# Mariachiar/Spatiotemporal-Deepfake-Detection-for-Live-Video-Calls

Measured on AMD Instinct MI355X. Metric: clips/sec (32x3x224x224), higher is better.
Workload: dtype bf16

## Files before the change

### spatiotemporal-deepfake-detection-for-live-video-calls_amd/csrc/af_conv.hip

```cpp
#include "af_common.h"
#include <stdlib.h>

namespace af {

#ifdef AF_STAMPS
#define AF_STAMP_DECL unsigned long long stamp_v[8] = {0, 0, 0, 0, 0, 0, 0, 0}
#define AF_DBG(bit) (a.dbg & (bit))
#define AF_STAMP(slot) stamp_v[slot] = (slot) >= 6 ? __builtin_amdgcn_s_memrealtime() : __builtin_amdgcn_s_memtime()
#define AF_STAMP_FLUSH do { if (a.stamps && lane < 8) a.stamps[((long long)bid * 8 + wave) * 8 + lane] = \
    lane == 0 ? stamp_v[0] : lane == 1 ? stamp_v[1] : lane == 2 ? stamp_v[2] : lane == 3 ? stamp_v[3] : lane == 4 ? stamp_v[4] : lane == 5 ? stamp_v[5] : lane == 6 ? stamp_v[6] : stamp_v[7]; } while (0)
#else
#define AF_STAMP_DECL do {} while (0)
#define AF_DBG(bit) false
#define AF_STAMP(slot) do {} while (0)
#define AF_STAMP_FLUSH do {} while (0)
#endif

struct ConvArgs {
    const char* in;
    const char* w;
    const float* scale;
    const float* shift;
    const char* res;
    char* out;
// ... 569 lines not shown
    conv_igemm_tile<DT, BN, BM, WN, WM, KS, NSTAGE, MINW, DUAL, SPLITK, BMR>(a, blockIdx.x, gridDim.x);
}

template <int DT, int BN, int BM, int WN, int WM, int KS, int MINW, bool DUAL, int NSTAGE = 3, bool SPLITK = false, int BMR = BM>
static int launch(const ConvArgs& a, hipStream_t stream) {
    const long long tiles_m = (a.M + BMR - 1) / BMR;
    const long long blocks = tiles_m * a.tiles_n;
    if (blocks <= 0 || blocks > 0x7fffffffLL) return set_error(AF_ERR_ARG, "conv: grid of %lld workgroups", blocks);
    constexpr int TMv = BMR / WM / 16;
    constexpr int red_bytes = KS == 2 ? WN * WM * (BN / WN / 16) * TMv * 64 * 16 : 0;
    constexpr int patch_bytes = red_bytes + WN * WM * ((TMv % 4 == 0 && TMv >= 8 ? TMv / 4 : TMv % 2 == 0 ? TMv / 2 : 1) * 16) * (BN / WN + 4) * 4;
    const int S = a.kt * a.kh * a.kw * a.kpt + a.kpt2;
    const int slots = (MINW >= 4 && a.ring == 2) ? 2 : NSTAGE;
    const int ring_bytes = (S < slots ? S : slots) * (BN + BM) * 128;
    const int lds = ring_bytes > patch_bytes ? ring_bytes : patch_bytes;
    AF_SET_MAX_LDS((&conv_igemm_kernel<DT, BN, BM, WN, WM, KS, NSTAGE, MINW, DUAL, SPLITK, BMR>),
                   NSTAGE * (BN + BM) * 128 > patch_bytes ? NSTAGE * (BN + BM) * 128 : patch_bytes, "conv");
    hipLaunchKernelGGL((conv_igemm_kernel<DT, BN, BM, WN, WM, KS, NSTAGE, MINW, DUAL, SPLITK, BMR>), dim3((unsigned)blocks, SPLITK ? a.ksplit : 1), dim3(WN * WM * KS * 64), lds, stream, a);
    AF_CHECK_LAUNCH("conv_igemm_kernel");
    return AF_OK;
}

enum { VAR_128x256 = 0, VAR_64x256 = 1, VAR_128x128 = 2, VAR_64x128 = 3, VAR_C133 = 4, VAR_128x128_R2 = 5, VAR_256x256 = 6,
       VAR_128x512 = 7, VAR_C311 = 8, VAR_SMALL = 9, VAR_C111 = 10, VAR_C133G = 11, VAR_256x224 = 12, VAR_C311G = 13, VAR_COUNT = 14 };
static const char* const kVariantNames[] = {"conv_igemm<BN=128,BM=256>", "conv_igemm<BN=64,BM=256>",
                                            "conv_igemm<BN=128,BM=128>", "conv_igemm<BN=64,BM=128>",
                                            "conv133_c64<weights in registers>", "conv_igemm<BN=128,BM=128>",
                                            "conv_igemm<BN=256,BM=256>", "conv_igemm<BN=128,BM=512>",
                                            "conv311_c64<time-tiled, taps share one LDS image>",
                                            "conv_small<direct-gather MFMA, narrow layers>",
                                            "conv111<persistent stream, weights in registers>",
                                            "conv133g<frame-resident halo patch, 9 taps share it>",
                                            "conv_igemm<BN=256,BM=224>",
                                            "conv311g<clip-resident (T + 2) x P patch, 3 taps share it>"};

static int pick_variant(int cout, int cin, int taps, int dtype, long long M, int cin2 = 0, int pooled = 0) {
    if (const char* fv = getenv("AF_FORCE_VAR")) {
        const int v = atoi(fv);
        const int bn = (v == VAR_256x256 || v == VAR_256x224) ? 256 : (v == VAR_128x256 || v == VAR_128x512 || v == VAR_128x128 || v == VAR_128x128_R2) ? 128 : 64;
        const bool generic = v == VAR_128x256 || v == VAR_64x256 || v == VAR_128x128 || v == VAR_64x128 || v == VAR_128x128_R2 ||
                             v == VAR_256x256 || v == VAR_128x512 || v == VAR_256x224;
        if (generic && cout % bn == 0 && !(pooled && v == VAR_256x224)) return v;
    }
    const int ksteps = (taps * cin + cin2) / (dtype == AF_F32 ? 32 : 64);
    const bool wide = cout % 128 == 0, short_k = ksteps <= 3;
    if (cout % 256 == 0 && ksteps >= (pooled == 2 ? 4 : cin2 ? 6 : 9)) {
        const char* e224 = getenv("AF_IGEMM_224");
        const int mode224 = e224 ? atoi(e224) : 1;
        const long long tm = (M + 255) / 256, big = tm * (cout / 256), v0 = tm * (cout / 128);
        const long long b224 = (M + 223) / 224 * (cout / 256);
        const double c256 = (double)((big + 255) / 256), c224 = 0.89 * (double)((b224 + 255) / 256);
        const bool take224 = pooled == 0 && mode224 != 0 && (mode224 == 2 || (M % 49 == 0 && c224 < c256 - 0.02));
        if (big >= 128 && (take224 ? c224 : c256) < 0.615 * (double)((v0 + 255) / 256) + 0.05) return take224 ? VAR_256x224 : VAR_256x256;
    }
    if (cout == 128 && !cin2 && taps >= 9) {
        const long long big = (M + 511) / 512, v0 = (M + 255) / 256;
        if (big >= 128 && (double)((big + 255) / 256) < 0.615 * (double)((v0 + 255) / 256) + 0.05) return VAR_128x512;
// ... 73 lines not shown
            case VAR_256x224: rc = launch<DT, 256, 256, 4, 2, 1, 2, false, 2, false, 224>(a, stream); break;
            case VAR_128x512: rc = launch<DT, 128, 512, 2, 4, 1, 2, false, 2>(a, stream); break;
            case VAR_128x256: rc = launch<DT, 128, 256, 2, 4, 1, 2, false>(a, stream); break;
            case VAR_64x256: rc = launch<DT, 64, 256, 1, 8, 1, 2, false>(a, stream); break;
            case VAR_128x128:
            case VAR_128x128_R2: rc = launch<DT, 128, 128, 2, 4, 1, 6, false>(a, stream); break;
            default: rc = launch<DT, 64, 128, 1, 8, 1, 4, false>(a, stream); break;
        }
    }
    if (rc != AF_OK || a.ksplit == 1) return rc;
    const long long quads = a.M * (a.Cout / 4);
    hipLaunchKernelGGL((splitk_finish_kernel<DT>), dim3((unsigned)((quads + 255) / 256)), dim3(256), 0, stream, a.ws, a.ksplit, a.M, a.Cout,
                       a.scale, a.shift, a.res, a.relu, a.out, a.out_ld);
    AF_CHECK_LAUNCH("splitk_finish_kernel");
    return AF_OK;
}

}

extern "C" int af_conv_variant(const af_conv_desc* d, const af_conv_desc* d2) {
    AF_REQUIRE(d && d->cout > 0 && d->cin > 0 && af::dtype_ok(d->dtype), "conv_variant: bad descriptor");
    if (af::conv_small_applies(d, d2, nullptr, 0)) return af::VAR_SMALL;
    if (!d2 && af::conv133_applies(d, nullptr, 0)) return af::VAR_C133;
    if (!d2 && af::conv133g_applies(d, nullptr, 0)) return af::VAR_C133G;
    if (!d2 && af::conv311g_applies(d, nullptr, 0)) return af::VAR_C311G;
    if (!d2 && af::conv311_applies(d, nullptr, 0)) return af::VAR_C311;
    if (af::conv111_applies(d, d2, nullptr, 0)) return af::VAR_C111;
    const int bk = d->dtype == AF_F32 ? 32 : 64;
    return af::pick_variant((d->cout + 63) / 64 * 64, (d->cin + bk - 1) / bk * bk, d->kt * d->kh * d->kw, d->dtype,
                            (long long)d->n * d->to * d->ho * d->wo, d2 ? (d2->cin + bk - 1) / bk * bk : 0, d->tpool);
}

extern "C" const char* af_conv_variant_name(int variant) {
    return (variant >= 0 && variant < af::VAR_COUNT) ? af::kVariantNames[variant] : "?";
}

extern "C" int64_t af_conv_workspace_bytes(const af_conv_desc* d) {
    using namespace af;
    if (!d || d->cout <= 0 || d->cin <= 0 || !dtype_ok(d->dtype) || d->n <= 0 || d->to <= 0 || d->ho <= 0 || d->wo <= 0) return 0;
    const int bk = d->dtype == AF_F32 ? 32 : 64;
    const int coutp = (d->cout + 63) / 64 * 64, cinp = (d->cin + bk - 1) / bk * bk, taps = d->kt * d->kh * d->kw;
    const long long M = (long long)d->n * d->to * d->ho * d->wo;
    const int v = pick_variant(coutp, cinp, taps, d->dtype, M, 0, d->tpool);
    const int ks = plan_ksplit(v, M, coutp, d->cout, taps * (cinp / bk), d->tpool, false);
    return ks > 1 ? (int64_t)ks * M * d->cout * (int64_t)sizeof(float) : 0;
}

// ... 146 lines not shown
```

### spatiotemporal-deepfake-detection-for-live-video-calls_amd/csrc/af_conv133g.hip

```cpp
#include "af_common.h"
#include <stdlib.h>

namespace af {

#ifdef AF_STAMPS
#define AF_STAMP_DECL unsigned long long stamp_v[8] = {0, 0, 0, 0, 0, 0, 0, 0}
#define AF_DBG(bit) (a.dbg & (bit))
#define AF_STAMP(slot) stamp_v[slot] = (slot) >= 6 ? __builtin_amdgcn_s_memrealtime() : __builtin_amdgcn_s_memtime()
#define AF_STAMP_FLUSH do { if (a.stamps && lane < 8) a.stamps[((long long)blockIdx.x * 8 + wave) * 8 + lane] = \
    lane == 0 ? stamp_v[0] : lane == 1 ? stamp_v[1] : lane == 2 ? stamp_v[2] : lane == 3 ? stamp_v[3] : lane == 4 ? stamp_v[4] : lane == 5 ? stamp_v[5] : lane == 6 ? stamp_v[6] : stamp_v[7]; } while (0)
#else
#define AF_STAMP_DECL do {} while (0)
#define AF_DBG(bit) false
#define AF_STAMP(slot) do {} while (0)
#define AF_STAMP_FLUSH do {} while (0)
#endif

struct C133GArgs {
    const char* in;
    const char* w;
    const float* scale;
    const float* shift;
    char* out;
    int H, W, Cin, Cout, frames;
    int T, kt;
    int R, upf;
    int WP;
    int prows;
    int kslabs;
    int relu, out_ld;
    float inv_wp;
    const char* w2;
    const float* scale2;
    const float* shift2;
    const char* res;
    int Cout2, relu2;
    int stagger;
#ifdef AF_STAMPS
    unsigned long long* stamps;
    int dbg;
#endif
};

template <int DT, int WN, int WM, int MT, bool FUSEC, int MAXP, int NSLOT, bool TEMPORAL>
__global__ __launch_bounds__(512, 2) void conv133g_kernel(const C133GArgs a) {
    typedef Elem<DT> E;
    typedef typename E::type OT;
    static_assert(E::EPC == 8 && WN * WM == 8, "16-bit operands, 8 waves");
    constexpr int NT = 4;
    constexpr int BN = WN * 64;
    constexpr int RW = BN / 64;
    constexpr int WSTAGE = BN * 128;
    constexpr int PROW = 64 + 8;
    constexpr int NTAPS = TEMPORAL ? 3 : 9;
    constexpr int PSTEPS = TEMPORAL ? NTAPS - 1 : NTAPS;
    constexpr int PPS = (MAXP + PSTEPS - 1) / PSTEPS;
    static_assert(!(TEMPORAL && FUSEC) && NSLOT <= NTAPS, "temporal mode: no fused c conv; the prologue's stages are taps of slab 0");

    extern __shared__ uint4 smem[];
    const unsigned lds0 = (unsigned)(uintptr_t)(__attribute__((address_space(3))) char*)smem;
    const int tid = threadIdx.x, lane = tid & 63;
    const int wave = __builtin_amdgcn_readfirstlane(tid >> 6);
    const int wn = wave % WN, wm = wave / WN;
    const int frow = lane & 15, fg = lane >> 4;
    const int WP = a.WP;
    const int pbytes = a.prows * 128;
    const unsigned ring0 = lds0 + 2 * pbytes;

    const int units = a.frames * a.upf;
    int unit = blockIdx.x;
    int frame = unit / a.upf, h0 = (unit - frame * a.upf) * a.R;
    const int HW = a.H * a.W;
    const int lrow = tid >> 3, wchunk = (tid & 7) ^ (lrow & 7);
    const long long Kw = (long long)NTAPS * a.kt * a.Cin;
    const i32x4 wdesc = make_desc(a.w);
    const unsigned woff = (unsigned)((lrow * Kw + wchunk * 8) * 2);
    const int wpiece_bytes = (int)(64 * Kw * 2);
    const int NP = a.prows >> 3;
    const int pt = a.kt >> 1;
    int tclip = frame % a.T;
    const int frame_bytes = a.H * a.W * a.Cin * 2;
    auto unit_desc = [&]() {
        return make_desc(TEMPORAL ? a.in + ((((long long)frame * a.T - 1) * HW + h0) * a.Cin) * 2
                                  : a.in + ((((long long)frame - pt) * a.H + h0 - 1) * a.W) * a.Cin * 2);
    };
    i32x4 xdesc = unit_desc();
    constexpr bool POFF_LDS = WN == 2;
    unsigned poff[POFF_LDS ? 1 : MAXP];
    const unsigned tab0 = ring0 + NSLOT * WSTAGE;
    const unsigned tabl = tab0 + (unsigned)((wave * 8 + (lane >> 3)) * 4);
    const unsigned pchunk16 = (unsigned)(((lane & 7) ^ (lane >> 3)) * 16);
    auto patch_slab_offset = [&](int ks, bool& inclip) {
        const int dt = (ks >= a.kslabs) + (ks >= 2 * a.kslabs), cs = ks - dt * a.kslabs;
        inclip = (unsigned)(tclip + dt - pt) < (unsigned)a.T;
        return __builtin_amdgcn_readfirstlane(dt * frame_bytes + cs * 128);
    };
    auto issue_patch_piece = [&](int bufoff, int soff, bool inclip, int i, unsigned voff) {
        if (wave + 8 * i < NP)
            blds16_m0(inclip ? voff : kOutOfRange, xdesc, soff, __builtin_amdgcn_readfirstlane(lds0 + bufoff + (wave + 8 * i) * 1024));
    };
    auto table_offset = [&](unsigned word) { return word == kOutOfRange ? kOutOfRange : word + pchunk16; };
    auto w_slab_offset = [&](int ks) {
        const int dt = (ks >= a.kslabs) + (ks >= 2 * a.kslabs), cs = ks - dt * a.kslabs;
        return __builtin_amdgcn_readfirstlane((dt * NTAPS * a.Cin + cs * 64) * 2);
    };
    const int tap_bytes = a.Cin * 2;
    auto issue_w_piece = [&](int stoff, int soff, int i) {
        blds16_m0(woff, wdesc, soff + i * wpiece_bytes, __builtin_amdgcn_readfirstlane(ring0 + stoff + (64 * i + 8 * wave) * 128));
    };

    f32x4 acc[NT][MT];

    const int nslabs = a.kt * a.kslabs;
    AF_STAMP_DECL;
    AF_STAMP(0); AF_STAMP(6);
    auto row_offset = [&](int j) -> unsigned {
        if (TEMPORAL) {
            const int tf = (int)(((float)j + 0.5f) * a.inv_wp), q = j - tf * a.R;
            const bool ok = tf >= 1 && tf <= a.T && h0 + q < HW;
            return ok ? (unsigned)((((long long)tf * HW + q) * a.Cin) * 2) : kOutOfRange;
        }
        const int q = j - 1;
        const int r = (int)(((float)q + 0.5f) * a.inv_wp), c = q - r * WP;
        const bool ok = q >= 0 && r < a.R + 2 && c >= 1 && c <= a.W && (unsigned)(h0 - 1 + r) < (unsigned)a.H;
        return ok ? (unsigned)(((r * a.W + (c - 1)) * a.Cin) * 2) : kOutOfRange;
    };
    auto compute_poff = [&]() {
        if constexpr (POFF_LDS) {
            int t = tid;
            asm volatile("" : "+v"(t));
            unsigned* tab = reinterpret_cast<unsigned*>(reinterpret_cast<char*>(smem) + (tab0 - lds0));
            for (int j = t; j < a.prows; j += 512) tab[j] = row_offset(j);
            asm volatile("s_waitcnt lgkmcnt(0)" ::: "memory");
            __builtin_amdgcn_s_barrier();
        } else {
            int drow = lane >> 3;
            asm volatile("" : "+v"(drow));
#pragma unroll
            for (int i = 0; i < MAXP; ++i) poff[i] = table_offset(row_offset((wave + 8 * i) * 8 + drow));
        }
    };
    auto issue_unit_head = [&](int bufoff) {
#pragma unroll
        for (int k = 0; k < NSLOT; ++k)
#pragma unroll
            for (int i = 0; i < RW; ++i) issue_w_piece(k * WSTAGE, w_slab_offset(0) + k * tap_bytes, i);
        compute_poff();
        bool in0;
        const int ps0 = patch_slab_offset(0, in0);
        if constexpr (POFF_LDS) {
            unsigned w[MAXP];
            static_for<MAXP>([&](auto i) { w[i] = lds_read4_uncounted<i * 256>(tabl); });
            wait_lgkmcnt<0>();
#pragma unroll
            for (int i = 0; i < MAXP; ++i) { asm volatile("" : "+v"(w[i])); issue_patch_piece(bufoff, ps0, in0, i, table_offset(w[i])); }
        } else {
#pragma unroll
            for (int i = 0; i < MAXP; ++i) issue_patch_piece(bufoff, ps0, in0, i, poff[i]);
        }
    };
    issue_unit_head(0);
    int bstart = 0;
    const unsigned arow = ring0 + (wn * 64 + frow) * 128, brow = lds0 + (wm * MT * 16 + frow) * 128;
    u32x4 a0[NT], b0[MT], a1[NT], b1[MT];
    auto frag_read = [&](u32x4 (&af)[NT], u32x4 (&bf)[MT], unsigned wsb, unsigned xsb, auto idx) {
        constexpr int r = decltype(idx)::value;
        if constexpr (r < NT) af[r] = lds_read16_uncounted<r * (16 * 128)>(wsb);
        else if constexpr (r < NT + MT) bf[r - NT] = lds_read16_uncounted<(r - NT) * (16 * 128)>(xsb);
    };
    auto w_addr = [&](int stoff, int kk) { return arow + stoff + ((((kk << 2) + fg) ^ (frow & 7)) << 4); };
    auto x_addr = [&](int bufoff, int sh, int kk) { return brow + bufoff + sh * 128 + ((((kk << 2) + fg) ^ ((frow + sh) & 7)) << 4); };
    auto pin_half = [&](u32x4 (&af)[NT], u32x4 (&bf)[MT]) {
#pragma unroll
        for (int i = 0; i < NT; ++i) pin_frag(af[i]);
#pragma unroll
        for (int j = 0; j < MT; ++j) pin_frag(bf[j]);
    };
    constexpr int NTH = NT * MT, NR = NT + MT;
    auto mma_group = [&](auto t0c, auto t1c, auto rlimc, const u32x4 (&af)[NT], const u32x4 (&bf)[MT], u32x4 (&naf)[NT], u32x4 (&nbf)[MT],
                         unsigned wsb, unsigned xsb) {
        constexpr int T0 = decltype(t0c)::value, T1 = decltype(t1c)::value, RLIM = decltype(rlimc)::value;
// ... 18 lines not shown
    for (;;) {
    wait_vmcnt<0>();
    __builtin_amdgcn_s_barrier();
#pragma unroll
    for (int i = 0; i < NT; ++i)
#pragma unroll
        for (int j = 0; j < MT; ++j) { acc[i][j] = f32x4{0.f, 0.f, 0.f, 0.f}; acc_live(acc[i][j]); }
    mfma_operands_settled();
    {
        constexpr int H1 = 3 * NTH / 4;
        static_assert(NR + RW + PPS <= NTH, "a DMA piece or a read per MFMA of the second group");
        int stoff = 0;
        int bufc = bstart, bufn = pbytes - bstart;
        {
            const unsigned wsb = w_addr(0, 0), xsb = x_addr(bufc, 0, 0);
            static_for<NR>([&](auto r) { frag_read(a0, b0, wsb, xsb, r); });
        }
        wait_lgkmcnt<0>();
        pin_half(a0, b0);
#pragma nounroll
        for (int slab = 0; slab < nslabs; ++slab) {
            const bool lastslab = slab + 1 == nslabs;
            const int wsl_c = w_slab_offset(slab), wsl_n = w_slab_offset(lastslab ? slab : slab + 1);
            bool in1;
            const int ps1 = patch_slab_offset(lastslab ? slab : slab + 1, in1);
            const bool pp = !lastslab;
            static_for<NTAPS>([&](auto tapc) {
                constexpr int tap = tapc, ntap = (tap + 1) % NTAPS;
                constexpr int t2 = (tap + NSLOT) % NTAPS;
                int sh = TEMPORAL ? tap * a.R : (tap / 3) * WP + tap % 3, nsh = TEMPORAL ? ntap * a.R : (ntap / 3) * WP + ntap % 3;
                asm volatile("" : "+s"(sh), "+s"(nsh));
                const unsigned wsb1 = w_addr(stoff, 1), xsb1 = x_addr(bufc, sh, 1);
                unsigned pw[PPS];
                if constexpr (POFF_LDS && tap < PSTEPS) {
                    static_for<PPS>([&](auto sl) {
                        constexpr int piece = tap * PPS + decltype(sl)::value;
                        if constexpr (piece < MAXP) pw[sl] = lds_read4_uncounted<piece * 256>(tabl);
                    });
                }
                const bool laststep = tap == NTAPS - 1 && lastslab;
                mma_group(IC<0>{}, IC<H1>{}, IC<H1>{}, a0, b0, a1, b1, wsb1, xsb1);
                auto wait_stage = [&]() {
                    if (AF_DBG(1)) return;
                    if (NSLOT == 2 || (tap - 1 + NSLOT >= NTAPS && lastslab)) wait_vmcnt<0>();
                    else wait_vmcnt<RW>();
                };
                if (late && !laststep) {
                    wait_lgkmcnt<0>();
                    wait_stage();
                    if (!AF_DBG(2)) __builtin_amdgcn_s_barrier();
                }
                mma_group(IC<H1>{}, IC<NTH>{}, IC<0>{}, a0, b0, a1, b1, 0u, 0u);
                wait_lgkmcnt<0>();
                if (!late && !laststep) {
                    wait_stage();
                    if (!AF_DBG(2)) __builtin_amdgcn_s_barrier();
                }
                pin_half(a1, b1);
                const int stnext = NSLOT == 2 ? (stoff ^ WSTAGE) : (stoff == (NSLOT - 1) * WSTAGE ? 0 : stoff + WSTAGE);
                const unsigned wsb0 = w_addr(stnext, 0), xsb0 = x_addr(tap == NTAPS - 1 ? bufn : bufc, nsh, 0);
                const bool refill = (tap + NSLOT < NTAPS || !lastslab) && !AF_DBG(4);
                const int wsoff = (tap + NSLOT < NTAPS ? wsl_c : wsl_n) + t2 * tap_bytes;
                static_for<NTH>([&](auto tc) {
                    constexpr int t = tc, slot = group2_slot(t, RW + PPS, NR);
                    MmaAsm<DT>::run(a1[t / MT], b1[t % MT], acc[t / MT][t % MT]);
                    if constexpr (slot != kNoSlot && slot < 0) frag_read(a0, b0, wsb0, xsb0, IC<-1 - slot>{});
                    else if constexpr (slot != kNoSlot && slot < PPS) {
                        constexpr int piece = tap * PPS + slot;
                        if constexpr (piece < MAXP && tap < PSTEPS) {
                            if (pp && !AF_DBG(16)) {
                                if constexpr (POFF_LDS) { asm volatile("" : "+v"(pw[slot])); issue_patch_piece(bufn, ps1, in1, piece, table_offset(pw[slot])); }
                                else issue_patch_piece(bufn, ps1, in1, piece, poff[piece]);
                            }
                        }
                    } else if constexpr (slot != kNoSlot) { if (refill) issue_w_piece(stoff, wsoff, slot - PPS); }
                });
                stoff = stnext;
                wait_lgkmcnt<0>();
                pin_half(a0, b0);
            });
            const int tb = bufc; bufc = bufn; bufn = tb;
        }
    }
    AF_STAMP(1);
    AF_STAMP(2);
    mfma_drain();

    asm volatile("s_waitcnt lgkmcnt(0)" ::: "memory");
    __builtin_amdgcn_s_barrier();
    if constexpr (FUSEC) break;
    int lane_e = lane;
    asm volatile("" : "+v"(lane_e));
    const int frow_e = lane_e & 15, fg_e = lane_e >> 4;
    f32x4 sc[NT], sf[NT];
    {
        uint4 scr[NT], sfr[NT];
#pragma unroll
        for (int i = 0; i < NT; ++i) {
            scr[i] = gload16_uncounted(a.scale + wn * 64 + i * 16 + fg_e * 4);
            sfr[i] = gload16_uncounted(a.shift + wn * 64 + i * 16 + fg_e * 4);
        }
        const int e_frame = frame, e_h0 = h0;
        const int next = unit + (int)gridDim.x;
        const bool has_next = PERSIST && next < units;
        int younger = 0;
        if (has_next) {
            unit = next;
            frame = unit / a.upf; h0 = (unit - frame * a.upf) * a.R; tclip = frame % a.T;
            xdesc = unit_desc();
            issue_unit_head(pbytes);
            bstart = pbytes;
            int np = (NP - wave + 7) >> 3;
            younger = NSLOT * RW + (np < MAXP ? np : MAXP);
        }
        wait_vmcnt_dyn<NSLOT * RW + MAXP>(younger);
#pragma unroll
        for (int i = 0; i < NT; ++i) {
            u32x4 t0 = __builtin_bit_cast(u32x4, scr[i]), t1 = __builtin_bit_cast(u32x4, sfr[i]);
            pin_frag(t0); pin_frag(t1);
            sc[i] = __builtin_bit_cast(f32x4, t0); sf[i] = __builtin_bit_cast(f32x4, t1);
        }
        epi_frame = e_frame; epi_h0 = e_h0; epi_more = has_next;
    }
    const int rr = lane_e >> 3, cc = (lane_e & 7) * 8;
    if (!FUSEC) {
        OT* patch = reinterpret_cast<OT*>(smem) + wave * (16 * PROW);
        char* obase = TEMPORAL ? a.out + (((long long)epi_frame * a.T) * HW + epi_h0) * a.out_ld * 2 + wn * 128
                               : a.out + (((long long)epi_frame * a.H + epi_h0) * a.W) * a.out_ld * 2 + wn * 128;
#pragma unroll
        for (int j = 0; j < MT; ++j) {
#pragma unroll
            for (int i = 0; i < NT; ++i) {
                f32x4 v = acc[i][j] * sc[i] + sf[i];
                if (a.relu) { v[0] = relu_f(v[0]); v[1] = relu_f(v[1]); v[2] = relu_f(v[2]); v[3] = relu_f(v[3]); }
                Vec4<DT>::store(reinterpret_cast<char*>(patch + frow_e * PROW + i * 16 + fg_e * 4), v);
            }
            __builtin_amdgcn_wave_barrier();
#pragma unroll
            for (int it = 0; it < 2; ++it) {
                const int row = it * 8 + rr;
                const int p = (wm * MT + j) * 16 + row;
                const int r = (int)(((float)p + 0.5f) * a.inv_wp), c = p - r * (TEMPORAL ? a.R : WP);
                const u32x4 o = *reinterpret_cast<const u32x4*>(patch + row * PROW + cc);
                if (TEMPORAL) {
                    if (r < a.T && epi_h0 + c < HW)
                        __builtin_nontemporal_store(o, reinterpret_cast<u32x4*>(obase + ((long long)r * HW + c) * a.out_ld * 2 + cc * 2));
                } else if (r < a.R && c >= 1 && c <= a.W && epi_h0 + r < a.H)
                    __builtin_nontemporal_store(o, reinterpret_cast<u32x4*>(obase + (long long)(r * a.W + c - 1) * a.out_ld * 2 + cc * 2));
            }
            __builtin_amdgcn_wave_barrier();
        }
        if (epi_more) continue;
        AF_STAMP(3); AF_STAMP(7);
        AF_STAMP_FLUSH;
        return;
    }
    }
    f32x4 sc[NT], sf[NT];
    const int frow_e = frow, fg_e = fg;
#pragma unroll
    for (int i = 0; i < NT; ++i) {
        sc[i] = *reinterpret_cast<const f32x4*>(a.scale + wn * 64 + i * 16 + fg_e * 4);
        sf[i] = *reinterpret_cast<const f32x4*>(a.shift + wn * 64 + i * 16 + fg_e * 4);
    }
    const int rr = lane >> 3, cc = (lane & 7) * 8;

    constexpr int MPAD = WM * MT * 16;
    char* T = reinterpret_cast<char*>(smem);
#pragma unroll
    for (int j = 0; j < MT; ++j) {
        const int p = (wm * MT + j) * 16 + frow_e;
// ... 56 lines not shown
                const f32x4 v0 = *reinterpret_cast<const f32x4*>(stg + row * SROW + cc);
                const f32x4 v1 = *reinterpret_cast<const f32x4*>(stg + row * SROW + cc + 4);
                if (r < a.R && c >= 1 && c <= a.W && h0 + r < a.H) {
                    const long long pix = pix0 + r * a.W + c - 1;
                    float v[8] = {v0[0], v0[1], v0[2], v0[3], v1[0], v1[1], v1[2], v1[3]};
                    if (a.res) {
                        const uint4 rraw = __builtin_bit_cast(uint4, __builtin_nontemporal_load(reinterpret_cast<const u32x4*>(a.res + (pix * a.Cout2 + ch0 + cc) * 2)));
                        const OT* re = reinterpret_cast<const OT*>(&rraw);
#pragma unroll
                        for (int e = 0; e < 8; ++e) v[e] += E::to_f32(re[e]);
                    }
                    uint4 o;
                    OT* oe = reinterpret_cast<OT*>(&o);
#pragma unroll
                    for (int e = 0; e < 8; ++e) oe[e] = E::from_f32(a.relu2 ? relu_f(v[e]) : v[e]);
                    __builtin_nontemporal_store(__builtin_bit_cast(u32x4, o), reinterpret_cast<u32x4*>(a.out + (pix * a.out_ld + ch0 + cc) * 2));
                }
            }
            __builtin_amdgcn_wave_barrier();
        }
    }
}

template <int DT, int WN, int WM, bool FUSEC, int MT, int MAXP, int NSLOT, bool TEMPORAL = false>
static int launch133g_n(const C133GArgs& a, hipStream_t stream) {
    if (a.prows > 64 * MAXP) return set_error(AF_ERR_ARG, "conv133g: %d patch rows for %d pieces per wave", a.prows, MAXP);
    int lds = 2 * a.prows * 128 + NSLOT * WN * 64 * 128 + (WN == 2 ? a.prows * 4 : 0);
    const int lds_c = WN * (WM * MT * 16) * 128 + 8 * 16 * (64 + 4) * 4;
    if (FUSEC && lds_c > lds) lds = lds_c;
    const int lds_e = 8 * 16 * (64 + 8) * 2;
    if (lds < lds_e) lds = lds_e;
    if (lds > 160 * 1024) return set_error(AF_ERR_ARG, "conv133g: %d bytes of LDS needed", lds);
    AF_SET_MAX_LDS((&conv133g_kernel<DT, WN, WM, MT, FUSEC, MAXP, NSLOT, TEMPORAL>), 160 * 1024, "conv133g");
    const int units = a.frames * a.upf, cus = device_cus();
    static const int persist = [] { const char* e = getenv("AF_G_PERSIST"); return e ? atoi(e) : 1; }();
    const int grid = (FUSEC || !persist || units <= cus || cus <= 0) ? units : cus;
    hipLaunchKernelGGL((conv133g_kernel<DT, WN, WM, MT, FUSEC, MAXP, NSLOT, TEMPORAL>), dim3(grid), dim3(512), lds, stream, a);
    AF_CHECK_LAUNCH("conv133g_kernel");
    return AF_OK;
}

template <int DT, int WN, int WM, bool FUSEC, int MT = 7, int MAXP = 9>
static int launch133g(const C133GArgs& a, hipStream_t stream) {
    if (!FUSEC && 2 * a.prows * 128 + 3 * WN * 64 * 128 + (WN == 2 ? a.prows * 4 : 0) <= 160 * 1024) return launch133g_n<DT, WN, WM, FUSEC, MT, MAXP, FUSEC ? 2 : 3>(a, stream);
    return launch133g_n<DT, WN, WM, FUSEC, MT, MAXP, 2>(a, stream);
}

static int conv133g_rows(const af_conv_desc* d) {
    if (d->dtype == AF_F32 || d->tpool) return 0;
    if ((d->kt != 1 && d->kt != 3) || d->kh != 3 || d->kw != 3 || d->st != 1 || d->sh != 1 || d->sw != 1) return 0;
    if (d->pt != d->kt / 2 || d->ph != 1 || d->pw != 1) return 0;
    if (d->cin % 64 != 0 || (d->cout != 128 && d->cout != 256 && !(d->cout == 64 && d->kt == 3))) return 0;
    const int mpad = d->cout == 256 ? 224 : d->cout == 128 ? 448 : 512;
    const int wp = d->w + 1;
    int r = mpad / wp;
    if (r > d->h) r = d->h;
    auto patch_rows = [&](int rows) { return ((rows + 2) * wp + 1 + 7) & ~7; };
    const int tab = d->cout == 128 ? 4 : 0;
    while (r >= 7 && (patch_rows(r) > 576 || 2 * patch_rows(r) * 128 + 2 * d->cout * 128 + patch_rows(r) * tab > 160 * 1024)) --r;
    if (r < 7) return 0;
    int upf = (d->h + r - 1) / r;
    r = (d->h + upf - 1) / upf;
    upf = (d->h + r - 1) / r;
    const long long units = (long long)d->n * d->t * upf;
    if (units < 192 || units > 0x7fffffffLL) return 0;
    if ((double)d->h * d->w / ((double)upf * mpad) < 0.6) return 0;
    if ((long long)(d->h + 2) * d->w * d->cin * 2 * (d->kt + 1) >= (1LL << 31)) return 0;
    return r;
}

bool conv133g_applies(const af_conv_desc* d, const void* residual, int out_ld) {
    return !residual && (out_ld == 0 || out_ld % 8 == 0) && conv133g_rows(d) != 0;
}

static void fill133g(C133GArgs& a, const af_conv_desc* d, const void* in, const void* w_packed, const float* scale,
                     const float* shift) {
    a.in = (const char*)in; a.w = (const char*)w_packed; a.scale = scale; a.shift = shift;
    a.H = d->h; a.W = d->w; a.Cin = d->cin; a.Cout = d->cout; a.frames = d->n * d->t;
    a.T = d->t; a.kt = d->kt;
    a.R = conv133g_rows(d); a.upf = (d->h + a.R - 1) / a.R; a.WP = d->w + 1;
    a.prows = ((a.R + 2) * a.WP + 1 + 7) & ~7;
    a.kslabs = d->cin / 64; a.relu = d->relu;
    a.inv_wp = 1.0f / (float)a.WP;
    a.w2 = nullptr; a.scale2 = a.shift2 = nullptr; a.res = nullptr; a.Cout2 = 0; a.relu2 = 0;
    const char* es = getenv("AF_G_STAGGER");
    a.stagger = es ? atoi(es) : 1;
#ifdef AF_STAMPS
    const char* ep = getenv("AF_STAMP_PTR");
    a.stamps = ep ? (unsigned long long*)strtoull(ep, nullptr, 0) : nullptr;
    const char* ed = getenv("AF_G_DBG");
    a.dbg = ed ? atoi(ed) : 0;
#endif
}

static int conv311g_pixels(const af_conv_desc* d) {
    if (d->dtype == AF_F32 || d->tpool) return 0;
    if (d->kt != 3 || d->kh != 1 || d->kw != 1 || d->st != 1 || d->sh != 1 || d->sw != 1) return 0;
    if (d->pt != 1 || d->ph != 0 || d->pw != 0) return 0;
    if (d->cin % 64 != 0 || (d->cout != 128 && d->cout != 256)) return 0;
    const int mpad = d->cout == 256 ? 224 : 448;
    if (d->t < 4 || mpad % d->t != 0) return 0;
    const int P = mpad / d->t;
    const int prows = ((d->t + 2) * P + 7) & ~7;
    if (P < 7 || prows > (d->cout == 256 ? 320 : 576) || 2 * prows * 128 + 2 * d->cout * 128 + (d->cout == 128 ? prows * 4 : 0) > 160 * 1024) return 0;
    const long long hw = (long long)d->h * d->w, chunks = (hw + P - 1) / P, units = (long long)d->n * chunks;
    if (units < 192 || units > 0x7fffffffLL) return 0;
    if ((double)hw / ((double)chunks * P) < 0.6) return 0;
    if ((long long)(d->t + 2) * hw * d->cin * 2 >= (1LL << 31)) return 0;
    return P;
}

bool conv311g_applies(const af_conv_desc* d, const void* residual, int out_ld) {
    static const int enabled = [] { const char* e = getenv("AF_T311G"); return e ? atoi(e) : 1; }();
    return enabled && !residual && (out_ld == 0 || out_ld % 8 == 0) && conv311g_pixels(d) != 0;
}

int conv311g_run(const af_conv_desc* d, const void* in, const void* w_packed, const float* scale, const float* shift,
                 void* out, int out_ld, hipStream_t stream) {
    C133GArgs a;
    a.in = (const char*)in; a.w = (const char*)w_packed; a.scale = scale; a.shift = shift;
    a.H = d->h; a.W = d->w; a.Cin = d->cin; a.Cout = d->cout; a.frames = d->n;
    a.T = d->t; a.kt = 1;
    a.R = conv311g_pixels(d); a.upf = (d->h * d->w + a.R - 1) / a.R; a.WP = a.R;
    a.prows = ((d->t + 2) * a.R + 7) & ~7;
    a.kslabs = d->cin / 64; a.relu = d->relu;
    a.inv_wp = 1.0f / (float)a.R;
    a.w2 = nullptr; a.scale2 = a.shift2 = nullptr; a.res = nullptr; a.Cout2 = 0; a.relu2 = 0;
    const char* es = getenv("AF_G_STAGGER");
    a.stagger = es ? atoi(es) : 1;
#ifdef AF_STAMPS
    const char* ep = getenv("AF_STAMP_PTR");
    a.stamps = ep ? (unsigned long long*)strtoull(ep, nullptr, 0) : nullptr;
    const char* ed = getenv("AF_G_DBG");
    a.dbg = ed ? atoi(ed) : 0;
#endif
    a.out = (char*)out; a.out_ld = out_ld ? out_ld : d->cout;
    const bool three = 2 * a.prows * 128 + 3 * d->cout * 128 + (d->cout == 128 ? a.prows * 4 : 0) <= 160 * 1024;
    if (d->cout == 256) {
        if (a.prows > 64 * 5) return set_error(AF_ERR_ARG, "conv311g: %d patch rows", a.prows);
        if (three) return d->dtype == AF_BF16 ? launch133g_n<AF_BF16, 4, 2, false, 7, 5, 3, true>(a, stream) : launch133g_n<AF_F16, 4, 2, false, 7, 5, 3, true>(a, stream);
        return d->dtype == AF_BF16 ? launch133g_n<AF_BF16, 4, 2, false, 7, 5, 2, true>(a, stream) : launch133g_n<AF_F16, 4, 2, false, 7, 5, 2, true>(a, stream);
    }
    if (three) return d->dtype == AF_BF16 ? launch133g_n<AF_BF16, 2, 4, false, 7, 9, 3, true>(a, stream) : launch133g_n<AF_F16, 2, 4, false, 7, 9, 3, true>(a, stream);
    return d->dtype == AF_BF16 ? launch133g_n<AF_BF16, 2, 4, false, 7, 9, 2, true>(a, stream) : launch133g_n<AF_F16, 2, 4, false, 7, 9, 2, true>(a, stream);
}

bool conv133g_fused_applies(const af_conv_desc* db, const af_conv_desc* dc, int out_ld) {
    if (!db || !dc || !conv133g_applies(db, nullptr, 0) || db->kt != 1 || db->cout == 64) return false;
    if (dc->dtype != db->dtype || dc->tpool || dc->kt != 1 || dc->kh != 1 || dc->kw != 1) return false;
    if (dc->st != 1 || dc->sh != 1 || dc->sw != 1 || dc->pt || dc->ph || dc->pw) return false;
    if (dc->n != db->n || dc->t != db->to || dc->h != db->ho || dc->w != db->wo || dc->cin != db->cout) return false;
    if (dc->cout % db->cout != 0) return false;
    return out_ld == 0 || (out_ld >= dc->cout && out_ld % 8 == 0);
}

int conv133g_fused_run(const af_conv_desc* db, const void* in, const void* wb, const float* scale_b, const float* shift_b,
                       const af_conv_desc* dc, const void* wc, const float* scale_c, const float* shift_c, const void* residual,
                       void* out, int out_ld, hipStream_t stream) {
    C133GArgs a;
    fill133g(a, db, in, wb, scale_b, shift_b);
    a.out = (char*)out; a.out_ld = out_ld ? out_ld : dc->cout;
    a.w2 = (const char*)wc; a.scale2 = scale_c; a.shift2 = shift_c; a.res = (const char*)residual; a.Cout2 = dc->cout; a.relu2 = dc->relu;
    if (db->cout == 256) return db->dtype == AF_BF16 ? launch133g<AF_BF16, 4, 2, true, 7, 5>(a, stream) : launch133g<AF_F16, 4, 2, true, 7, 5>(a, stream);
    return db->dtype == AF_BF16 ? launch133g<AF_BF16, 2, 4, true>(a, stream) : launch133g<AF_F16, 2, 4, true>(a, stream);
}

int conv133g_run(const af_conv_desc* d, const void* in, const void* w_packed, const float* scale, const float* shift,
                 void* out, int out_ld, hipStream_t stream) {
    C133GArgs a;
    fill133g(a, d, in, w_packed, scale, shift);
    a.out = (char*)out; a.out_ld = out_ld ? out_ld : d->cout;
    if (d->cout == 256) return d->dtype == AF_BF16 ? launch133g<AF_BF16, 4, 2, false, 7, 5>(a, stream) : launch133g<AF_F16, 4, 2, false, 7, 5>(a, stream);
    if (d->cout == 64) return d->dtype == AF_BF16 ? launch133g<AF_BF16, 1, 8, false, 4>(a, stream) : launch133g<AF_F16, 1, 8, false, 4>(a, stream);
    if (a.prows <= 512) return d->dtype == AF_BF16 ? launch133g<AF_BF16, 2, 4, false, 7, 8>(a, stream) : launch133g<AF_F16, 2, 4, false, 7, 8>(a, stream);
    return d->dtype == AF_BF16 ? launch133g<AF_BF16, 2, 4, false>(a, stream) : launch133g<AF_F16, 2, 4, false>(a, stream);
}

}
```

Measured before the change: 3500.

## Add stride-2 conv133g path using four parity-plane halo patches shared by taps

Extends the frame-resident halo-patch 3x3 conv kernel to handle stride-2 spatial convolutions by splitting the input into four parity planes (even/odd row and column). Each plane's patch is staged in LDS and shared by the 4/2/2/1 taps that read it, with tap reordering, per-plane masking and carried patch loads across buffers. Stride-2 3x3 layers (cout 128/256) previously went to the generic implicit-GEMM path; this aims to cut their redundant global gathers. The cost is considerably more complex scheduling and LDS buffer juggling, with the usual correctness risk at edges and odd sizes.

Result: no change. 3523 (median of 6 runs) (+0.7%).

```diff
diff --git a/spatiotemporal-deepfake-detection-for-live-video-calls_amd/csrc/af_conv.hip b/spatiotemporal-deepfake-detection-for-live-video-calls_amd/csrc/af_conv.hip
--- a/spatiotemporal-deepfake-detection-for-live-video-calls_amd/csrc/af_conv.hip
+++ b/spatiotemporal-deepfake-detection-for-live-video-calls_amd/csrc/af_conv.hip
@@ -615,7 +615,7 @@
 }
 
 enum { VAR_128x256 = 0, VAR_64x256 = 1, VAR_128x128 = 2, VAR_64x128 = 3, VAR_C133 = 4, VAR_128x128_R2 = 5, VAR_256x256 = 6,
-       VAR_128x512 = 7, VAR_C311 = 8, VAR_SMALL = 9, VAR_C111 = 10, VAR_C133G = 11, VAR_256x224 = 12, VAR_C311G = 13, VAR_COUNT = 14 };
+       VAR_128x512 = 7, VAR_C311 = 8, VAR_SMALL = 9, VAR_C111 = 10, VAR_C133G = 11, VAR_256x224 = 12, VAR_C311G = 13, VAR_C133G_S2 = 14, VAR_COUNT = 15 };
 static const char* const kVariantNames[] = {"conv_igemm<BN=128,BM=256>", "conv_igemm<BN=64,BM=256>",
                                             "conv_igemm<BN=128,BM=128>", "conv_igemm<BN=64,BM=128>",
                                             "conv133_c64<weights in registers>", "conv_igemm<BN=128,BM=128>",
@@ -625,7 +625,8 @@
                                             "conv111<persistent stream, weights in registers>",
                                             "conv133g<frame-resident halo patch, 9 taps share it>",
                                             "conv_igemm<BN=256,BM=224>",
-                                            "conv311g<clip-resident (T + 2) x P patch, 3 taps share it>"};
+                                            "conv311g<clip-resident (T + 2) x P patch, 3 taps share it>",
+                                            "conv133g_s2<four parity-plane halo patches, 4/2/2/1 taps share one>"};
 
 static int pick_variant(int cout, int cin, int taps, int dtype, long long M, int cin2 = 0, int pooled = 0) {
     if (const char* fv = getenv("AF_FORCE_VAR")) {
@@ -745,7 +746,7 @@
     AF_REQUIRE(d && d->cout > 0 && d->cin > 0 && af::dtype_ok(d->dtype), "conv_variant: bad descriptor");
     if (af::conv_small_applies(d, d2, nullptr, 0)) return af::VAR_SMALL;
     if (!d2 && af::conv133_applies(d, nullptr, 0)) return af::VAR_C133;
-    if (!d2 && af::conv133g_applies(d, nullptr, 0)) return af::VAR_C133G;
+    if (!d2 && af::conv133g_applies(d, nullptr, 0)) return d->sh == 2 ? af::VAR_C133G_S2 : af::VAR_C133G;
     if (!d2 && af::conv311g_applies(d, nullptr, 0)) return af::VAR_C311G;
     if (!d2 && af::conv311_applies(d, nullptr, 0)) return af::VAR_C311;
     if (af::conv111_applies(d, d2, nullptr, 0)) return af::VAR_C111;
diff --git a/spatiotemporal-deepfake-detection-for-live-video-calls_amd/csrc/af_conv133g.hip b/spatiotemporal-deepfake-detection-for-live-video-calls_amd/csrc/af_conv133g.hip
--- a/spatiotemporal-deepfake-detection-for-live-video-calls_amd/csrc/af_conv133g.hip
+++ b/spatiotemporal-deepfake-detection-for-live-video-calls_amd/csrc/af_conv133g.hip
@@ -23,6 +23,7 @@
     const float* shift;
     char* out;
     int H, W, Cin, Cout, frames;
+    int Ho, Wo;
     int T, kt;
     int R, upf;
     int WP;
@@ -42,7 +43,14 @@
 #endif
 };
 
-template <int DT, int WN, int WM, int MT, bool FUSEC, int MAXP, int NSLOT, bool TEMPORAL>
+__host__ __device__ constexpr int s2_tap(int k) { return k < 4 ? (k & 1) * 2 + (k >> 1) * 6 : k < 6 ? 3 + (k - 4) * 2 : k < 8 ? 1 + (k - 6) * 6 : 4; }
+__host__ __device__ constexpr int s2_plane(int k) { return k < 4 ? 0 : k < 6 ? 1 : k < 8 ? 2 : 3; }
+__host__ __device__ constexpr int s2_mask(int pl) { return (pl == 0 || pl == 2 ? 1 : 0) | (pl <= 1 ? 2 : 0); }
+__host__ __device__ constexpr int s2_carry(int k) { return k < 3 ? 1 : k < 5 ? 2 : k < 7 ? 3 : k == 7 ? 0 : -1; }
+__host__ __device__ constexpr int s2_cfirst(int k) { return k < 3 ? 0 : k < 5 ? 3 : k < 7 ? 5 : 7; }
+__host__ __device__ constexpr int s2_csteps(int k) { return k < 3 ? 3 : k < 7 ? 2 : 1; }
+
+template <int DT, int WN, int WM, int MT, bool FUSEC, int MAXP, int NSLOT, bool TEMPORAL, bool S2>
 __global__ __launch_bounds__(512, 2) void conv133g_kernel(const C133GArgs a) {
     typedef Elem<DT> E;
     typedef typename E::type OT;
@@ -54,8 +62,9 @@
     constexpr int PROW = 64 + 8;
     constexpr int NTAPS = TEMPORAL ? 3 : 9;
     constexpr int PSTEPS = TEMPORAL ? NTAPS - 1 : NTAPS;
-    constexpr int PPS = (MAXP + PSTEPS - 1) / PSTEPS;
+    constexpr int PPS = S2 ? MAXP : (MAXP + PSTEPS - 1) / PSTEPS;
     static_assert(!(TEMPORAL && FUSEC) && NSLOT <= NTAPS, "temporal mode: no fused c conv; the prologue's stages are taps of slab 0");
+    static_assert(!(S2 && (TEMPORAL || FUSEC)), "stride-2 mode: spatial, no fused c conv");
 
     extern __shared__ uint4 smem[];
     const unsigned lds0 = (unsigned)(uintptr_t)(__attribute__((address_space(3))) char*)smem;
@@ -82,6 +91,7 @@
     const int frame_bytes = a.H * a.W * a.Cin * 2;
     auto unit_desc = [&]() {
         return make_desc(TEMPORAL ? a.in + ((((long long)frame * a.T - 1) * HW + h0) * a.Cin) * 2
+                         : S2 ? a.in + (long long)frame * HW * a.Cin * 2
                                   : a.in + ((((long long)frame - pt) * a.H + h0 - 1) * a.W) * a.Cin * 2);
     };
     i32x4 xdesc = unit_desc();
@@ -100,6 +110,10 @@
             blds16_m0(inclip ? voff : kOutOfRange, xdesc, soff, __builtin_amdgcn_readfirstlane(lds0 + bufoff + (wave + 8 * i) * 1024));
     };
     auto table_offset = [&](unsigned word) { return word == kOutOfRange ? kOutOfRange : word + pchunk16; };
+    auto plane_voff = [&](unsigned v, int pl) { return (v & (kOutOfRange | (unsigned)s2_mask(pl))) ? kOutOfRange : v & ~3u; };
+    auto plane_soff = [&](int pl) {
+        return __builtin_amdgcn_readfirstlane(((s2_mask(pl) & 1) * a.W + (s2_mask(pl) >> 1)) * a.Cin * 2);
+    };
     auto w_slab_offset = [&](int ks) {
         const int dt = (ks >= a.kslabs) + (ks >= 2 * a.kslabs), cs = ks - dt * a.kslabs;
         return __builtin_amdgcn_readfirstlane((dt * NTAPS * a.Cin + cs * 64) * 2);
@@ -119,6 +133,14 @@
             const int tf = (int)(((float)j + 0.5f) * a.inv_wp), q = j - tf * a.R;
             const bool ok = tf >= 1 && tf <= a.T && h0 + q < HW;
             return ok ? (unsigned)((((long long)tf * HW + q) * a.Cin) * 2) : kOutOfRange;
+        }
+        if (S2) {
+            const int q = j - 1;
+            const int r = (int)(((float)q + 0.5f) * a.inv_wp), c = q - r * WP;
+            const int pr = h0 - 1 + r, pc = c - 1;
+            const bool ok = q >= 0 && r <= a.R && c >= 1 && pr >= 0 && 2 * pr < a.H;
+            return ok ? (unsigned)((2 * pr * a.W + 2 * pc) * a.Cin * 2) | (2 * pr + 1 >= a.H ? 1u : 0u) | (2 * pc + 1 >= a.W ? 2u : 0u)
+                      : kOutOfRange;
         }
         const int q = j - 1;
         const int r = (int)(((float)q + 0.5f) * a.inv_wp), c = q - r * WP;
@@ -144,19 +166,22 @@
 #pragma unroll
         for (int k = 0; k < NSLOT; ++k)
 #pragma unroll
-            for (int i = 0; i < RW; ++i) issue_w_piece(k * WSTAGE, w_slab_offset(0) + k * tap_bytes, i);
+            for (int i = 0; i < RW; ++i) issue_w_piece(k * WSTAGE, w_slab_offset(0) + (S2 ? s2_tap(k) : k) * tap_bytes, i);
         compute_poff();
         bool in0;
-        const int ps0 = patch_slab_offset(0, in0);
+        const int ps0 = patch_slab_offset(0, in0) + (S2 ? plane_soff(0) : 0);
         if constexpr (POFF_LDS) {
             unsigned w[MAXP];
             static_for<MAXP>([&](auto i) { w[i] = lds_read4_uncounted<i * 256>(tabl); });
             wait_lgkmcnt<0>();
 #pragma unroll
-            for (int i = 0; i < MAXP; ++i) { asm volatile("" : "+v"(w[i])); issue_patch_piece(bufoff, ps0, in0, i, table_offset(w[i])); }
+            for (int i = 0; i < MAXP; ++i) {
+                asm volatile("" : "+v"(w[i]));
+                issue_patch_piece(bufoff, ps0, in0, i, S2 ? plane_voff(table_offset(w[i]), 0) : table_offset(w[i]));
+            }
         } else {
 #pragma unroll
-            for (int i = 0; i < MAXP; ++i) issue_patch_piece(bufoff, ps0, in0, i, poff[i]);
+            for (int i = 0; i < MAXP; ++i) issue_patch_piece(bufoff, ps0, in0, i, S2 ? plane_voff(poff[i], 0) : poff[i]);
         }
     };
     issue_unit_head(0);
@@ -221,19 +246,28 @@
         for (int slab = 0; slab < nslabs; ++slab) {
             const bool lastslab = slab + 1 == nslabs;
             const int wsl_c = w_slab_offset(slab), wsl_n = w_slab_offset(lastslab ? slab : slab + 1);
-            bool in1;
+            bool in1, inc;
             const int ps1 = patch_slab_offset(lastslab ? slab : slab + 1, in1);
+            const int psc = S2 ? patch_slab_offset(slab, inc) : 0;
             const bool pp = !lastslab;
             static_for<NTAPS>([&](auto tapc) {
                 constexpr int tap = tapc, ntap = (tap + 1) % NTAPS;
                 constexpr int t2 = (tap + NSLOT) % NTAPS;
-                int sh = TEMPORAL ? tap * a.R : (tap / 3) * WP + tap % 3, nsh = TEMPORAL ? ntap * a.R : (ntap / 3) * WP + ntap % 3;
+                constexpr int wt = S2 ? s2_tap(tap) : tap, nwt = S2 ? s2_tap(ntap) : ntap, wt2 = S2 ? s2_tap(t2) : t2;
+                constexpr int CPL = S2 ? s2_carry(tap) : -1, CPG = S2 ? (MAXP + s2_csteps(tap) - 1) / s2_csteps(tap) : PPS;
+                constexpr int CP0 = S2 ? (tap - s2_cfirst(tap)) * CPG : tap * PPS;
+                constexpr int NPC = !S2 ? PPS : CPL < 0 ? 0 : (MAXP - CP0 < CPG ? MAXP - CP0 : CPG);
+                int sh = TEMPORAL ? tap * a.R : S2 ? (wt >= 3) * WP + (wt % 3 != 0) : (tap / 3) * WP + tap % 3,
+                    nsh = TEMPORAL ? ntap * a.R : S2 ? (nwt >= 3) * WP + (nwt % 3 != 0) : (ntap / 3) * WP + ntap % 3;
                 asm volatile("" : "+s"(sh), "+s"(nsh));
-                const unsigned wsb1 = w_addr(stoff, 1), xsb1 = x_addr(bufc, sh, 1);
-                unsigned pw[PPS];
-                if constexpr (POFF_LDS && tap < PSTEPS) {
-                    static_for<PPS>([&](auto sl) {
-                        constexpr int piece = tap * PPS + decltype(sl)::value;
+                int xbuf = S2 && (s2_plane(tap) & 1) ? bufn : bufc;
+                int nxbuf = S2 ? ((s2_plane(ntap) & 1) ? bufn : bufc) : tap == NTAPS - 1 ? bufn : bufc;
+                if constexpr (S2) asm volatile("" : "+s"(xbuf), "+s"(nxbuf));
+                const unsigned wsb1 = w_addr(stoff, 1), xsb1 = x_addr(xbuf, sh, 1);
+                unsigned pw[NPC > 0 ? NPC : 1];
+                if constexpr (POFF_LDS && tap < PSTEPS && NPC > 0) {
+                    static_for<NPC>([&](auto sl) {
+                        constexpr int piece = CP0 + decltype(sl)::value;
                         if constexpr (piece < MAXP) pw[sl] = lds_read4_uncounted<piece * 256>(tabl);
                     });
                 }
@@ -257,28 +291,33 @@
                 }
                 pin_half(a1, b1);
                 const int stnext = NSLOT == 2 ? (stoff ^ WSTAGE) : (stoff == (NSLOT - 1) * WSTAGE ? 0 : stoff + WSTAGE);
-                const unsigned wsb0 = w_addr(stnext, 0), xsb0 = x_addr(tap == NTAPS - 1 ? bufn : bufc, nsh, 0);
+                const unsigned wsb0 = w_addr(stnext, 0), xsb0 = x_addr(nxbuf, nsh, 0);
                 const bool refill = (tap + NSLOT < NTAPS || !lastslab) && !AF_DBG(4);
-                const int wsoff = (tap + NSLOT < NTAPS ? wsl_c : wsl_n) + t2 * tap_bytes;
+                const int wsoff = (tap + NSLOT < NTAPS ? wsl_c : wsl_n) + wt2 * tap_bytes;
+                const int cbuf = S2 ? ((CPL & 1) ? bufn : bufc) : bufn;
+                const int csoff = S2 ? (CPL == 0 ? ps1 : psc) + plane_soff(CPL < 0 ? 0 : CPL) : ps1;
+                const bool cpp = S2 ? (CPL != 0 || pp) : pp;
                 static_for<NTH>([&](auto tc) {
-                    constexpr int t = tc, slot = group2_slot(t, RW + PPS, NR);
+                    constexpr int t = tc, slot = group2_slot(t, RW + NPC, NR);
                     MmaAsm<DT>::run(a1[t / MT], b1[t % MT], acc[t / MT][t % MT]);
                     if constexpr (slot != kNoSlot && slot < 0) frag_read(a0, b0, wsb0, xsb0, IC<-1 - slot>{});
-                    else if constexpr (slot != kNoSlot && slot < PPS) {
-                        constexpr int piece = tap * PPS + slot;
+                    else if constexpr (slot != kNoSlot && slot < NPC) {
+                        constexpr int piece = CP0 + slot;
                         if constexpr (piece < MAXP && tap < PSTEPS) {
-                            if (pp && !AF_DBG(16)) {
-                                if constexpr (POFF_LDS) { asm volatile("" : "+v"(pw[slot])); issue_patch_piece(bufn, ps1, in1, piece, table_offset(pw[slot])); }
-                                else issue_patch_piece(bufn, ps1, in1, piece, poff[piece]);
+                            if (cpp && !AF_DBG(16)) {
+                                unsigned v;
+                                if constexpr (POFF_LDS) { asm volatile("" : "+v"(pw[slot])); v = table_offset(pw[slot]); }
+                                else { v = poff[piece]; if constexpr (S2) asm volatile("" : "+v"(v)); }
+                                issue_patch_piece(cbuf, csoff, in1, piece, S2 ? plane_voff(v, CPL < 0 ? 0 : CPL) : v);
                             }
                         }
-                    } else if constexpr (slot != kNoSlot) { if (refill) issue_w_piece(stoff, wsoff, slot - PPS); }
+                    } else if constexpr (slot != kNoSlot) { if (refill) issue_w_piece(stoff, wsoff, slot - NPC); }
                 });
                 stoff = stnext;
                 wait_lgkmcnt<0>();
                 pin_half(a0, b0);
             });
-            const int tb = bufc; bufc = bufn; bufn = tb;
+            if constexpr (!S2) { const int tb = bufc; bufc = bufn; bufn = tb; }
         }
     }
     AF_STAMP(1);
@@ -325,7 +364,7 @@
     if (!FUSEC) {
         OT* patch = reinterpret_cast<OT*>(smem) + wave * (16 * PROW);
         char* obase = TEMPORAL ? a.out + (((long long)epi_frame * a.T) * HW + epi_h0) * a.out_ld * 2 + wn * 128
-                               : a.out + (((long long)epi_frame * a.H + epi_h0) * a.W) * a.out_ld * 2 + wn * 128;
+                               : a.out + (((long long)epi_frame * a.Ho + epi_h0) * a.Wo) * a.out_ld * 2 + wn * 128;
 #pragma unroll
         for (int j = 0; j < MT; ++j) {
 #pragma unroll
@@ -344,8 +383,8 @@
                 if (TEMPORAL) {
                     if (r < a.T && epi_h0 + c < HW)
                         __builtin_nontemporal_store(o, reinterpret_cast<u32x4*>(obase + ((long long)r * HW + c) * a.out_ld * 2 + cc * 2));
-                } else if (r < a.R && c >= 1 && c <= a.W && epi_h0 + r < a.H)
-                    __builtin_nontemporal_store(o, reinterpret_cast<u32x4*>(obase + (long long)(r * a.W + c - 1) * a.out_ld * 2 + cc * 2));
+                } else if (r < a.R && c >= 1 && c <= a.Wo && epi_h0 + r < a.Ho)
+                    __builtin_nontemporal_store(o, reinterpret_cast<u32x4*>(obase + (long long)(r * a.Wo + c - 1) * a.out_ld * 2 + cc * 2));
             }
             __builtin_amdgcn_wave_barrier();
         }
@@ -448,7 +487,7 @@
     }
 }
 
-template <int DT, int WN, int WM, bool FUSEC, int MT, int MAXP, int NSLOT, bool TEMPORAL = false>
+template <int DT, int WN, int WM, bool FUSEC, int MT, int MAXP, int NSLOT, bool TEMPORAL = false, bool S2 = false>
 static int launch133g_n(const C133GArgs& a, hipStream_t stream) {
     if (a.prows > 64 * MAXP) return set_error(AF_ERR_ARG, "conv133g: %d patch rows for %d pieces per wave", a.prows, MAXP);
     int lds = 2 * a.prows * 128 + NSLOT * WN * 64 * 128 + (WN == 2 ? a.prows * 4 : 0);
@@ -457,40 +496,54 @@
     const int lds_e = 8 * 16 * (64 + 8) * 2;
     if (lds < lds_e) lds = lds_e;
     if (lds > 160 * 1024) return set_error(AF_ERR_ARG, "conv133g: %d bytes of LDS needed", lds);
-    AF_SET_MAX_LDS((&conv133g_kernel<DT, WN, WM, MT, FUSEC, MAXP, NSLOT, TEMPORAL>), 160 * 1024, "conv133g");
+    AF_SET_MAX_LDS((&conv133g_kernel<DT, WN, WM, MT, FUSEC, MAXP, NSLOT, TEMPORAL, S2>), 160 * 1024, "conv133g");
     const int units = a.frames * a.upf, cus = device_cus();
     static const int persist = [] { const char* e = getenv("AF_G_PERSIST"); return e ? atoi(e) : 1; }();
     const int grid = (FUSEC || !persist || units <= cus || cus <= 0) ? units : cus;
-    hipLaunchKernelGGL((conv133g_kernel<DT, WN, WM, MT, FUSEC, MAXP, NSLOT, TEMPORAL>), dim3(grid), dim3(512), lds, stream, a);
+    hipLaunchKernelGGL((conv133g_kernel<DT, WN, WM, MT, FUSEC, MAXP, NSLOT, TEMPORAL, S2>), dim3(grid), dim3(512), lds, stream, a);
     AF_CHECK_LAUNCH("conv133g_kernel");
     return AF_OK;
 }
 
-template <int DT, int WN, int WM, bool FUSEC, int MT = 7, int MAXP = 9>
+template <int DT, int WN, int WM, bool FUSEC, int MT = 7, int MAXP = 9, bool S2 = false>
 static int launch133g(const C133GArgs& a, hipStream_t stream) {
-    if (!FUSEC && 2 * a.prows * 128 + 3 * WN * 64 * 128 + (WN == 2 ? a.prows * 4 : 0) <= 160 * 1024) return launch133g_n<DT, WN, WM, FUSEC, MT, MAXP, FUSEC ? 2 : 3>(a, stream);
-    return launch133g_n<DT, WN, WM, FUSEC, MT, MAXP, 2>(a, stream);
+    if (!FUSEC && 2 * a.prows * 128 + 3 * WN * 64 * 128 + (WN == 2 ? a.prows * 4 : 0) <= 160 * 1024) return launch133g_n<DT, WN, WM, FUSEC, MT, MAXP, FUSEC ? 2 : 3, false, S2>(a, stream);
+    return launch133g_n<DT, WN, WM, FUSEC, MT, MAXP, 2, false, S2>(a, stream);
+}
+
+static bool conv133g_s2_enabled() {
+    static const int enabled = [] { const char* e = getenv("AF_G_S2"); return e ? atoi(e) : 1; }();
+    return enabled != 0;
+}
+
+static int conv133g_stagger() {
+    static const int stagger = [] { const char* e = getenv("AF_G_STAGGER"); return e ? atoi(e) : 1; }();
+    return stagger;
 }
 
 static int conv133g_rows(const af_conv_desc* d) {
     if (d->dtype == AF_F32 || d->tpool) return 0;
-    if ((d->kt != 1 && d->kt != 3) || d->kh != 3 || d->kw != 3 || d->st != 1 || d->sh != 1 || d->sw != 1) return 0;
+    const bool s2 = d->sh == 2 && d->sw == 2;
+    if ((d->kt != 1 && d->kt != 3) || d->kh != 3 || d->kw != 3 || d->st != 1 || !((d->sh == 1 && d->sw == 1) || s2)) return 0;
     if (d->pt != d->kt / 2 || d->ph != 1 || d->pw != 1) return 0;
+    if (s2 && (d->kt != 1 || d->cout == 64 || !conv133g_s2_enabled())) return 0;
     if (d->cin % 64 != 0 || (d->cout != 128 && d->cout != 256 && !(d->cout == 64 && d->kt == 3))) return 0;
     const int mpad = d->cout == 256 ? 224 : d->cout == 128 ? 448 : 512;
-    const int wp = d->w + 1;
+    const int ho = s2 ? d->ho : d->h, wo = s2 ? d->wo : d->w;
+    const int wp = wo + 1;
     int r = mpad / wp;
-    if (r > d->h) r = d->h;
-    auto patch_rows = [&](int rows) { return ((rows + 2) * wp + 1 + 7) & ~7; };
+    if (r > ho) r = ho;
+    auto patch_rows = [&](int rows) { return ((rows + (s2 ? 1 : 2)) * wp + 1 + 7) & ~7; };
+    const int maxrows = s2 ? (d->cout == 256 ? 320 : 512) : 576;
     const int tab = d->cout == 128 ? 4 : 0;
-    while (r >= 7 && (patch_rows(r) > 576 || 2 * patch_rows(r) * 128 + 2 * d->cout * 128 + patch_rows(r) * tab > 160 * 1024)) --r;
+    while (r >= 7 && (patch_rows(r) > maxrows || 2 * patch_rows(r) * 128 + 2 * d->cout * 128 + patch_rows(r) * tab > 160 * 1024)) --r;
     if (r < 7) return 0;
-    int upf = (d->h + r - 1) / r;
-    r = (d->h + upf - 1) / upf;
-    upf = (d->h + r - 1) / r;
+    int upf = (ho + r - 1) / r;
+    r = (ho + upf - 1) / upf;
+    upf = (ho + r - 1) / r;
     const long long units = (long long)d->n * d->t * upf;
     if (units < 192 || units > 0x7fffffffLL) return 0;
-    if ((double)d->h * d->w / ((double)upf * mpad) < 0.6) return 0;
+    if ((double)ho * wo / ((double)upf * mpad) < 0.6) return 0;
     if ((long long)(d->h + 2) * d->w * d->cin * 2 * (d->kt + 1) >= (1LL << 31)) return 0;
     return r;
 }
@@ -502,15 +555,16 @@
 static void fill133g(C133GArgs& a, const af_conv_desc* d, const void* in, const void* w_packed, const float* scale,
                      const float* shift) {
     a.in = (const char*)in; a.w = (const char*)w_packed; a.scale = scale; a.shift = shift;
+    const bool s2 = d->sh == 2;
     a.H = d->h; a.W = d->w; a.Cin = d->cin; a.Cout = d->cout; a.frames = d->n * d->t;
+    a.Ho = s2 ? d->ho : d->h; a.Wo = s2 ? d->wo : d->w;
     a.T = d->t; a.kt = d->kt;
-    a.R = conv133g_rows(d); a.upf = (d->h + a.R - 1) / a.R; a.WP = d->w + 1;
-    a.prows = ((a.R + 2) * a.WP + 1 + 7) & ~7;
+    a.R = conv133g_rows(d); a.upf = (a.Ho + a.R - 1) / a.R; a.WP = a.Wo + 1;
+    a.prows = ((a.R + (s2 ? 1 : 2)) * a.WP + 1 + 7) & ~7;
     a.kslabs = d->cin / 64; a.relu = d->relu;
     a.inv_wp = 1.0f / (float)a.WP;
     a.w2 = nullptr; a.scale2 = a.shift2 = nullptr; a.res = nullptr; a.Cout2 = 0; a.relu2 = 0;
-    const char* es = getenv("AF_G_STAGGER");
-    a.stagger = es ? atoi(es) : 1;
+    a.stagger = conv133g_stagger();
 #ifdef AF_STAMPS
     const char* ep = getenv("AF_STAMP_PTR");
     a.stamps = ep ? (unsigned long long*)strtoull(ep, nullptr, 0) : nullptr;
@@ -546,14 +600,14 @@
     C133GArgs a;
     a.in = (const char*)in; a.w = (const char*)w_packed; a.scale = scale; a.shift = shift;
     a.H = d->h; a.W = d->w; a.Cin = d->cin; a.Cout = d->cout; a.frames = d->n;
+    a.Ho = d->h; a.Wo = d->w;
     a.T = d->t; a.kt = 1;
     a.R = conv311g_pixels(d); a.upf = (d->h * d->w + a.R - 1) / a.R; a.WP = a.R;
     a.prows = ((d->t + 2) * a.R + 7) & ~7;
     a.kslabs = d->cin / 64; a.relu = d->relu;
     a.inv_wp = 1.0f / (float)a.R;
     a.w2 = nullptr; a.scale2 = a.shift2 = nullptr; a.res = nullptr; a.Cout2 = 0; a.relu2 = 0;
-    const char* es = getenv("AF_G_STAGGER");
-    a.stagger = es ? atoi(es) : 1;
+    a.stagger = conv133g_stagger();
 #ifdef AF_STAMPS
     const char* ep = getenv("AF_STAMP_PTR");
     a.stamps = ep ? (unsigned long long*)strtoull(ep, nullptr, 0) : nullptr;
@@ -572,7 +626,7 @@
 }
 
 bool conv133g_fused_applies(const af_conv_desc* db, const af_conv_desc* dc, int out_ld) {
-    if (!db || !dc || !conv133g_applies(db, nullptr, 0) || db->kt != 1 || db->cout == 64) return false;
+    if (!db || !dc || !conv133g_applies(db, nullptr, 0) || db->kt != 1 || db->cout == 64 || db->sh != 1) return false;
     if (dc->dtype != db->dtype || dc->tpool || dc->kt != 1 || dc->kh != 1 || dc->kw != 1) return false;
     if (dc->st != 1 || dc->sh != 1 || dc->sw != 1 || dc->pt || dc->ph || dc->pw) return false;
     if (dc->n != db->n || dc->t != db->to || dc->h != db->ho || dc->w != db->wo || dc->cin != db->cout) return false;
@@ -596,6 +650,10 @@
     C133GArgs a;
     fill133g(a, d, in, w_packed, scale, shift);
     a.out = (char*)out; a.out_ld = out_ld ? out_ld : d->cout;
+    if (d->sh == 2) {
+        if (d->cout == 256) return d->dtype == AF_BF16 ? launch133g<AF_BF16, 4, 2, false, 7, 5, true>(a, stream) : launch133g<AF_F16, 4, 2, false, 7, 5, true>(a, stream);
+        return d->dtype == AF_BF16 ? launch133g<AF_BF16, 2, 4, false, 7, 8, true>(a, stream) : launch133g<AF_F16, 2, 4, false, 7, 8, true>(a, stream);
+    }
     if (d->cout == 256) return d->dtype == AF_BF16 ? launch133g<AF_BF16, 4, 2, false, 7, 5>(a, stream) : launch133g<AF_F16, 4, 2, false, 7, 5>(a, stream);
     if (d->cout == 64) return d->dtype == AF_BF16 ? launch133g<AF_BF16, 1, 8, false, 4>(a, stream) : launch133g<AF_F16, 1, 8, false, 4>(a, stream);
     if (a.prows <= 512) return d->dtype == AF_BF16 ? launch133g<AF_BF16, 2, 4, false, 7, 8>(a, stream) : launch133g<AF_F16, 2, 4, false, 7, 8>(a, stream);
```
